# KELVIN-ASU/Lightweight-Multi-Modal-Scene-Understanding-via-Knowledge-Distillation

Measured on AMD Instinct MI355X. Metric: PandaSet 2-class KD training frames/sec, higher is better.
Workload: dtype f32; 1 GPU; KD step: concat-fusion teacher fwd (eval) -> weighted-fusion student fwd/bwd (train BN), CE + T^2*KL(T=4) + feature-MSE, fused AdamW; random-init weights; teacher_fusion=concat, student_fusion=weighted, image=3x256x256, points_per_frame=80000, bev_grid=64x64, num_classes=2, per_gpu_batch=256, global_batch=256, parallelism=dp1

## Files before the change

lightweight-multi-modal-scene-understanding-via-knowledge-distillation_amd/csrc/kd_lidar.hip:

```cpp
#include "kd_common.h"

namespace {

struct BevGeom { float x0, xd, y0, yd; int H, W; };

__device__ __forceinline__ bool bev_cell(const float4 pt, const BevGeom g, int& cell) {
  const float xn = __fdiv_rn(__fsub_rn(pt.x, g.x0), g.xd);
  const float yn = __fdiv_rn(__fsub_rn(pt.y, g.y0), g.yd);
  const bool valid = (xn >= 0.f) && (xn <= 1.f) && (yn >= 0.f) && (yn <= 1.f);
  if (!valid) { cell = -1; return false; }
  long long ix = (long long)__fmul_rn(xn, (float)(g.W - 1));
  long long iy = (long long)__fmul_rn(yn, (float)(g.H - 1));
  ix = ix < 0 ? 0 : (ix > g.W - 1 ? g.W - 1 : ix);
  iy = iy < 0 ? 0 : (iy > g.H - 1 ? g.H - 1 : iy);
  cell = (int)(iy * g.W + ix);
  return true;
}

struct L0Args {
  const float* pts; const float* w; const float* b; float* y; float* partial;
  int64_t P; int C; int groups, slots; const int* p_dev;
};
__global__ __launch_bounds__(256) void lidar_l0_fwd_kernel(L0Args a) {
  __shared__ float red[2 * 256 * 4];
// ... 290 lines not shown
  if (lane == 0) wave_cnt[wave] = __popcll(m);
  __syncthreads();
  if (threadIdx.x == 0) {
    int tot = 0;
    for (int w = 0; w < (int)(blockDim.x >> 6); ++w) { wave_off[w] = tot; tot += wave_cnt[w]; }
    block_base = tot ? atomicAdd(counter, tot) : 0;
  }
  __syncthreads();
  if (valid) {
    const int idx = block_base + wave_off[wave] + before;
    kd_st4(out_pts + (int64_t)idx * 4, pt);
    out_cell[idx] = (int)(p / N) * (g.H * g.W) + c;
  }
}
int kd_lidar_compact(const float* pts, float* out_pts, int* out_cell, int* counter, int B, int64_t N, int H, int W,
                     float x0, float x1, float y0, float y1, void* stream) {
  KD_REQUIRE(pts && out_pts && out_cell && counter && B > 0 && N > 0, KD_ERR_ARG, "kd_lidar_compact: bad args");
  hipStream_t st = (hipStream_t)stream;
  hipError_t e = kd_fill_async(counter, 0, sizeof(int), st);
  KD_REQUIRE(e == hipSuccess, (int)e, "kd_lidar_compact: memset failed: %s", hipGetErrorString(e));
  const int64_t P = (int64_t)B * N;
  hipLaunchKernelGGL(lidar_compact_kernel, dim3((unsigned)((P + 1023) / 1024)), dim3(1024), 0, st, pts, out_pts, out_cell,
                     counter, P, N, BevGeom{x0, x1 - x0, y0, y1 - y0, H, W});
  return kd_check_launch("kd_lidar_compact");
}

__global__ __launch_bounds__(256) void scatter_max_idx_kernel(const float* __restrict__ y, const float* __restrict__ sc,
                                                              const float* __restrict__ sh, int act,
                                                              const int* __restrict__ cell_idx, float* grid, int64_t P, int C,
                                                              int groups, int slots, const int* p_dev) {
  const int tid = threadIdx.x;
  const int gidx = tid % groups, slot = tid / groups;
  if (slot >= slots) return;
  const int G = groups;
  float s[4], h[4];
#pragma unroll
  for (int j = 0; j < 4; ++j) { s[j] = sc[gidx + G * j]; h[j] = sh[gidx + G * j]; }
  if (p_dev) { const int64_t pv = *p_dev; P = pv < P ? pv : P; }
  for (int64_t p = (int64_t)blockIdx.x * slots + slot; p < P; p += (int64_t)gridDim.x * slots) {
    const float* yp = y + p * C + gidx;
    unsigned* dst = reinterpret_cast<unsigned*>(grid + (int64_t)cell_idx[p] * C + gidx);
    float v[4];
    unsigned cur[4];
#pragma unroll
    for (int j = 0; j < 4; ++j) { v[j] = kd_act(kd_affine(yp[G * j], s[j], h[j]), act); cur[j] = dst[G * j]; }
#pragma unroll
    for (int j = 0; j < 4; ++j) {
      const unsigned u = __float_as_uint(v[j]);
      if (v[j] > 0.f && u > cur[j]) atomicMax(dst + G * j, u);
    }
  }
}
int kd_lidar_scatter_max_idx_fwd(const float* y, const float* sc, const float* sh, int act, const int* cell_idx,
                                 float* grid, int64_t P, int C, int64_t ncells, const int* p_dev, void* stream) {
  KD_REQUIRE(y && sc && sh && cell_idx && grid && P >= 0 && C % 4 == 0 && C <= 1024 && ncells > 0, KD_ERR_ARG, "kd_lidar_scatter_max_idx_fwd: bad args");
  KD_REQUIRE(act == KD_ACT_RELU || act == KD_ACT_RELU6, KD_ERR_ARG, "kd_lidar_scatter_max_idx_fwd: needs a non-negative activation");
  hipStream_t st = (hipStream_t)stream;
  hipError_t e = kd_fill_async(grid, 0, (size_t)ncells * C * sizeof(float), st);
  KD_REQUIRE(e == hipSuccess, (int)e, "kd_lidar_scatter_max_idx_fwd: memset failed: %s", hipGetErrorString(e));
  if (P == 0) return KD_OK;
  const KdCgLayout l = kd_cg_layout(P, C, 4096);
  hipLaunchKernelGGL(scatter_max_idx_kernel, dim3(l.grid), dim3(256), 0, st, y, sc, sh, act, cell_idx, grid, P, C, l.groups,
                     l.slots, p_dev);
  return kd_check_launch("kd_lidar_scatter_max_idx_fwd");
}

}

namespace {

constexpr int SCAN_CHUNK = 2048;

__global__ void seg_count_kernel(const float* __restrict__ pts, int* __restrict__ row_of_point, int* __restrict__ rank,
                                 int* counts, int64_t P, int64_t N, BevGeom g) {
  const int64_t p = (int64_t)blockIdx.x * blockDim.x + threadIdx.x;
  if (p >= P) return;
  int c;
  if (bev_cell(kd_ld4(pts + p * 4), g, c)) {
    const int row = (int)(p / N) * (g.H * g.W) + c;
    row_of_point[p] = row;
    rank[p] = atomicAdd(counts + row, 1);
  } else {
    row_of_point[p] = -1;
  }
}

__global__ __launch_bounds__(256) void scan_block_sums_kernel(const int* __restrict__ v, int* __restrict__ bsum, int64_t n) {
  __shared__ int red[256];
  const int64_t base = (int64_t)blockIdx.x * SCAN_CHUNK;
  int s = 0;
  for (int i = threadIdx.x; i < SCAN_CHUNK; i += 256)
    if (base + i < n) s += v[base + i];
  red[threadIdx.x] = s;
  __syncthreads();
  for (int off = 128; off > 0; off >>= 1) {
    if ((int)threadIdx.x < off) red[threadIdx.x] += red[threadIdx.x + off];
    __syncthreads();
  }
  if (threadIdx.x == 0) bsum[blockIdx.x] = red[0];
}

__global__ __launch_bounds__(1024) void scan_bsums_kernel(int* bsum, int nb) {
  __shared__ int sh[1024];
  int carry = 0;
  for (int base = 0; base < nb; base += 1024) {
    const int i = base + (int)threadIdx.x;
    const int v = i < nb ? bsum[i] : 0;
    sh[threadIdx.x] = v;
    __syncthreads();
    for (int off = 1; off < 1024; off <<= 1) {
      const int t = (int)threadIdx.x >= off ? sh[threadIdx.x - off] : 0;
      __syncthreads();
      sh[threadIdx.x] += t;
      __syncthreads();
    }
    if (i < nb) bsum[i] = carry + sh[threadIdx.x] - v;
    carry += sh[1023];
    __syncthreads();
  }
}

__global__ __launch_bounds__(256) void scan_apply_kernel(int* v, const int* __restrict__ bsum, int64_t n) {
  __shared__ int sh[256];
  const int64_t base = (int64_t)blockIdx.x * SCAN_CHUNK + (int64_t)threadIdx.x * 8;
  int x[8];
  int tot = 0;
#pragma unroll
  for (int j = 0; j < 8; ++j) { x[j] = base + j < n ? v[base + j] : 0; tot += x[j]; }
  sh[threadIdx.x] = tot;
  __syncthreads();
  for (int off = 1; off < 256; off <<= 1) {
    const int t = (int)threadIdx.x >= off ? sh[threadIdx.x - off] : 0;
    __syncthreads();
    sh[threadIdx.x] += t;
    __syncthreads();
  }
  int run = bsum[blockIdx.x] + sh[threadIdx.x] - tot;
#pragma unroll
  for (int j = 0; j < 8; ++j) {
    if (base + j < n) v[base + j] = run;
    run += x[j];
  }
}

__global__ void seg_fill_kernel(const int* __restrict__ row_of_point, const int* __restrict__ rank,
                                const int* __restrict__ start, int* __restrict__ perm, int64_t P) {
  const int64_t p = (int64_t)blockIdx.x * blockDim.x + threadIdx.x;
  if (p >= P) return;
  const int row = row_of_point[p];
  if (row >= 0) perm[start[row] + rank[p]] = (int)p;
}

constexpr int SORT_BLK = 1024;
constexpr int SORT_MAX_BINS = 36865;

__global__ __launch_bounds__(SORT_BLK) void stable_count_kernel(const float* __restrict__ pts, int* __restrict__ key_out,
                                                                int* __restrict__ lrank_out, int* __restrict__ T, int64_t N,
                                                                int nblk, BevGeom g) {
  extern __shared__ int hist[];
  const int HW = g.H * g.W, nb = HW + 1;
  const int tid = threadIdx.x, lane = tid & 63, wave = tid >> 6;
  const int b = blockIdx.x / nblk, blk = blockIdx.x % nblk;
  for (int i = tid; i < nb; i += SORT_BLK) hist[i] = 0;
  const int64_t n = (int64_t)blk * SORT_BLK + tid;
  const bool act = n < N;
  const int64_t p = (int64_t)b * N + (act ? n : 0);
  int key = -1;
  if (act) {
    int c;
    key = bev_cell(kd_ld4(pts + p * 4), g, c) ? c : HW;
  }
  int r = 0, cnt = 0;
#pragma unroll 16
  for (int j = 0; j < 64; ++j) {
    const int kj = __shfl(key, j);
    cnt += kj == key ? 1 : 0;
    r += (kj == key && j < lane) ? 1 : 0;
  }
  __syncthreads();
  int lr = 0;
  for (int w = 0; w < SORT_BLK / 64; ++w) {
    if (wave == w && act) lr = hist[key] + r;
    __syncthreads();
    if (wave == w && act && r == cnt - 1) hist[key] += cnt;
    __syncthreads();
  }
  if (act) { key_out[p] = key; lrank_out[p] = lr; }
  int* Tb = T + ((int64_t)b * nblk + blk) * nb;
  for (int i = tid; i < nb; i += SORT_BLK) Tb[i] = hist[i];
}

__global__ void stable_prefix_kernel(int* T, int* __restrict__ counts, int* __restrict__ inv, int B, int nblk, int HW) {
  const int nb = HW + 1;
  const int64_t idx = (int64_t)blockIdx.x * blockDim.x + threadIdx.x;
  if (idx == 0) counts[(int64_t)B * HW] = 0;
  if (idx >= (int64_t)B * nb) return;
  const int b = (int)(idx / nb), key = (int)(idx % nb);
  int run = 0;
  for (int blk = 0; blk < nblk; ++blk) {
    int* t = T + ((int64_t)b * nblk + blk) * nb + key;
    const int v = *t;
    *t = run;
    run += v;
  }
  if (key < HW) counts[(int64_t)b * HW + key] = run; else inv[b] = run;
}

__global__ void stable_inv_base_kernel(const int* __restrict__ seg_start, int* inv, int B, int64_t ncells) {
  if (threadIdx.x != 0 || blockIdx.x != 0) return;
  int run = seg_start[ncells];
  for (int b = 0; b < B; ++b) { const int v = inv[b]; inv[b] = run; run += v; }
}

__global__ void stable_fill_kernel(const float* __restrict__ pts, const int* __restrict__ key, const int* __restrict__ lrank,
                                   const int* __restrict__ T, const int* __restrict__ seg_start, const int* __restrict__ inv_base,
                                   float* __restrict__ pts_sorted, int* __restrict__ row_sorted, int* __restrict__ perm,
                                   int64_t P, int64_t N, int nblk, int HW) {
  const int64_t p = (int64_t)blockIdx.x * blockDim.x + threadIdx.x;
  if (p >= P) return;
  const int b = (int)(p / N), blk = (int)((p % N) / SORT_BLK), k = key[p];
  const int base = k < HW ? seg_start[(int64_t)b * HW + k] : inv_base[b];
  const int64_t pos = (int64_t)base + T[((int64_t)b * nblk + blk) * (HW + 1) + k] + lrank[p];
  kd_st4(pts_sorted + pos * 4, kd_ld4(pts + p * 4));
  row_sorted[pos] = k < HW ? b * HW + k : -1;
  if (perm) perm[pos] = (int)p;
}

constexpr int WIDE_MAX_DIM = 4096;

__device__ __forceinline__ void wave_same_key(int key, int lane, int& below, int& all) {
  below = 0; all = 0;
#pragma unroll 16
  for (int j = 0; j < 64; ++j) {
    const int kj = __shfl(key, j);
    all += kj == key ? 1 : 0;
    below += (kj == key && j < lane) ? 1 : 0;
  }
}

__device__ __forceinline__ int block_stable_rank(int key, bool act, int below, int all, int* hist) {
  const int wave = threadIdx.x >> 6;
  int lr = 0;
  for (int w = 0; w < SORT_BLK / 64; ++w) {
    if (wave == w && act) lr = hist[key] + below;
    __syncthreads();
    if (wave == w && act && below == all - 1) hist[key] += all;
    __syncthreads();
  }
  return lr;
}

template <int PASS>
__global__ __launch_bounds__(SORT_BLK) void wide_count_kernel(const float* __restrict__ pts, int* __restrict__ cell_io,
                                                              int* __restrict__ lrank_out, int* __restrict__ T,
                                                              int* counts, int64_t N, int nblk, BevGeom g) {
  extern __shared__ int hist[];
  const int nd = PASS == 0 ? g.W : g.H + 1;
  const int tid = threadIdx.x, lane = tid & 63;
  const int b = blockIdx.x / nblk, blk = blockIdx.x % nblk;
  for (int i = tid; i < nd; i += SORT_BLK) hist[i] = 0;
  const int64_t n = (int64_t)blk * SORT_BLK + tid;
  const bool act = n < N;
  const int64_t p = (int64_t)b * N + (act ? n : 0);
  int cell = -1;
  if (act) {
    if (PASS == 0) bev_cell(kd_ld4(pts + p * 4), g, cell); else cell = cell_io[p];
  }
  const int key = !act ? -1 : PASS == 0 ? (cell >= 0 ? cell % g.W : 0) : (cell >= 0 ? cell / g.W : g.H);
  int below, all;
  wave_same_key(key, lane, below, all);
  if (PASS == 0) {
    int cbelow, call;
    wave_same_key(cell, lane, cbelow, call);
    if (cell >= 0 && cbelow == 0) atomicAdd(counts + (int64_t)b * g.H * g.W + cell, call);
  }
  __syncthreads();
  const int lr = block_stable_rank(key, act, below, all, hist);
  if (act) {
    if (PASS == 0) cell_io[p] = cell;
    lrank_out[p] = lr;
  }
  int* Tb = T + ((int64_t)b * nblk + blk) * nd;
  for (int i = tid; i < nd; i += SORT_BLK) Tb[i] = hist[i];
}

__global__ void wide_prefix_kernel(int* T, int* __restrict__ tot, int* __restrict__ last_tot, int B, int nblk, int nd) {
  const int64_t idx = (int64_t)blockIdx.x * blockDim.x + threadIdx.x;
  if (idx >= (int64_t)B * nd) return;
  const int b = (int)(idx / nd), d = (int)(idx % nd);
  int run = 0;
  for (int blk = 0; blk < nblk; ++blk) {
    int* t = T + ((int64_t)b * nblk + blk) * nd + d;
    const int v = *t;
    *t = run;
    run += v;
  }
  tot[idx] = run;
  if (last_tot && d == nd - 1) last_tot[b] = run;
}

__global__ __launch_bounds__(64) void wide_frame_scan_kernel(int* tot, int nd) {
  int* t = tot + (int64_t)blockIdx.x * nd;
  const int lane = threadIdx.x;
  int carry = 0;
  for (int base = 0; base < nd; base += 64) {
    const int i = base + lane;
    const int v = i < nd ? t[i] : 0;
    int incl = v;
#pragma unroll
    for (int off = 1; off < 64; off <<= 1) {
      const int u = __shfl_up(incl, off);
      if (lane >= off) incl += u;
    }
    if (i < nd) t[i] = carry + incl - v;
    carry += __shfl(incl, 63);
  }
}

__global__ void wide_mid_kernel(const int* __restrict__ cell, const int* __restrict__ lrank, const int* __restrict__ T,
                                const int* __restrict__ off, int* __restrict__ mid_id, int* __restrict__ mid_cell, int64_t P,
                                int64_t N, int nblk, int W) {
  const int64_t p = (int64_t)blockIdx.x * blockDim.x + threadIdx.x;
  if (p >= P) return;
  const int b = (int)(p / N), blk = (int)((p % N) / SORT_BLK), c = cell[p];
  const int d = c >= 0 ? c % W : 0;
  const int64_t pos = (int64_t)b * N + off[(int64_t)b * W + d] + T[((int64_t)b * nblk + blk) * W + d] + lrank[p];
  mid_id[pos] = (int)p;
  mid_cell[pos] = c;
}

__global__ void wide_fill_kernel(const float* __restrict__ pts, const int* __restrict__ mid_id, const int* __restrict__ mid_cell,
                                 const int* __restrict__ lrank, const int* __restrict__ T, const int* __restrict__ off,
                                 const int* __restrict__ seg_start, const int* __restrict__ inv_base,
                                 float* __restrict__ pts_sorted, int* __restrict__ row_sorted, int* __restrict__ perm,
                                 int64_t P, int64_t N, int nblk, int H, int W) {
  const int64_t q = (int64_t)blockIdx.x * blockDim.x + threadIdx.x;
  if (q >= P) return;
  const int b = (int)(q / N), blk = (int)((q % N) / SORT_BLK), c = mid_cell[q], p = mid_id[q];
  const int nd = H + 1, d = c >= 0 ? c / W : H;
  const int64_t HW = (int64_t)H * W;
  const int in_digit = T[((int64_t)b * nblk + blk) * nd + d] + lrank[q];
  const int64_t pos = c >= 0 ? (int64_t)seg_start[b * HW] + off[(int64_t)b * nd + d] + in_digit : (int64_t)inv_base[b] + in_digit;
  kd_st4(pts_sorted + pos * 4, kd_ld4(pts + (int64_t)p * 4));
  row_sorted[pos] = c >= 0 ? (int)(b * HW + c) : -1;
  if (perm) perm[pos] = p;
}

struct SegArgs {
  const float* y; const float* sc; const float* sh; int act;
  const int* start; const int* perm;
  float* grid; const float* dout; const float* mean; const float* invstd;
  float* G; float* partial; int64_t ncells; int C;
  int long_len; const int* rowid; float* cnt; int prow0;
  float* rawmax; uint8_t* holders;
};
constexpr int SEG_LONG = 256;
constexpr int SEG_HOLD_SWEEP = 255;

template <int VEC> struct SegVec;
template <> struct SegVec<1> { typedef float type; };
template <> struct SegVec<2> { typedef float2 type; };
template <> struct SegVec<4> { typedef float4 type; };

template <int VEC> __device__ __forceinline__ void seg_ld(float (&r)[VEC], const float* p) {
  const typename SegVec<VEC>::type v = *reinterpret_cast<const typename SegVec<VEC>::type*>(p);
  __builtin_memcpy(r, &v, sizeof(v));
}
template <int VEC> __device__ __forceinline__ void seg_st(float* p, const float (&r)[VEC]) {
  typename SegVec<VEC>::type v;
  __builtin_memcpy(&v, r, sizeof(v));
  *reinterpret_cast<typename SegVec<VEC>::type*>(p) = v;
}

template <int VEC, bool PERM>
__global__ __launch_bounds__(256) void seg_max_fwd_kernel(SegArgs a) {
  const int lane = threadIdx.x & 63;
// ... 305 lines not shown
  const int nvalid = __builtin_amdgcn_readfirstlane(a.start[a.ncells]);
  const int64_t nw = (int64_t)gridDim.x * 4;
  for (int64_t w = (int64_t)blockIdx.x * 4 + wave; w * 64 < nvalid; w += nw) {
    const int i0 = (int)(w * 64), i1 = i0 + 64 < nvalid ? i0 + 64 : nvalid;
    const int cf = __builtin_amdgcn_readfirstlane(a.rowid[i0]), cl = __builtin_amdgcn_readfirstlane(a.rowid[i1 - 1]);
    const bool lf = a.start[cf + 1] - a.start[cf] > a.long_len, ll = a.start[cl + 1] - a.start[cl] > a.long_len;
    if (!lf && !ll) continue;
    int i = i0;
    while (i < i1) {
      const int cell = __builtin_amdgcn_readfirstlane(a.rowid[i]);
      const int cs = __builtin_amdgcn_readfirstlane(a.start[cell]), ce = __builtin_amdgcn_readfirstlane(a.start[cell + 1]);
      const int rend = ce < i1 ? ce : i1;
      if (ce - cs <= a.long_len) { i = rend; continue; }
      float acc[VEC], mx[VEC], share[VEC];
#pragma unroll
      for (int j = 0; j < VEC; ++j) { acc[j] = 0.f; mx[j] = 0.f; share[j] = 0.f; }
      if (MODE >= 1) seg_ld<VEC>(mx, a.grid + (int64_t)cell * a.C + c0);
      if (MODE == 2) {
        float d[VEC], n[VEC];
        seg_ld<VEC>(d, a.dout + (int64_t)cell * a.C + c0);
        seg_ld<VEC>(n, a.cnt + (int64_t)cell * a.C + c0);
#pragma unroll
        for (int j = 0; j < VEC; ++j) share[j] = n[j] > 0.f ? d[j] / n[j] : 0.f;
        if (i == cs) seg_st<VEC>(a.G + (int64_t)cell * a.C + c0, share);
      }
      int k = i;
      for (; k + 4 <= rend; k += 4) {
        float r[4][VEC];
#pragma unroll
        for (int u = 0; u < 4; ++u) seg_ld<VEC>(r[u], a.y + (int64_t)(k + u) * a.C + c0);
#pragma unroll
        for (int u = 0; u < 4; ++u)
#pragma unroll
          for (int j = 0; j < VEC; ++j) {
            const float v = kd_act(kd_affine(r[u][j], sc[j], sh[j]), a.act);
            if (MODE == 0) acc[j] = v > acc[j] ? v : acc[j];
            if (MODE == 1) acc[j] += (v > 0.f && v == mx[j]) ? 1.f : 0.f;
            if (MODE == 2) {
              const float g = (v > 0.f && v == mx[j]) ? share[j] : 0.f;
              s1[j] += g;
              s2[j] = fmaf(g, (r[u][j] - mu[j]) * inv[j], s2[j]);
            }
          }
      }
      for (; k < rend; ++k) {
        float r[VEC];
        seg_ld<VEC>(r, a.y + (int64_t)k * a.C + c0);
#pragma unroll
        for (int j = 0; j < VEC; ++j) {
          const float v = kd_act(kd_affine(r[j], sc[j], sh[j]), a.act);
          if (MODE == 0) acc[j] = v > acc[j] ? v : acc[j];
          if (MODE == 1) acc[j] += (v > 0.f && v == mx[j]) ? 1.f : 0.f;
          if (MODE == 2) {
            const float g = (v > 0.f && v == mx[j]) ? share[j] : 0.f;
            s1[j] += g;
            s2[j] = fmaf(g, (r[j] - mu[j]) * inv[j], s2[j]);
          }
        }
      }
      if (MODE == 0) {
        unsigned* dst = reinterpret_cast<unsigned*>(a.grid + (int64_t)cell * a.C + c0);
#pragma unroll
        for (int j = 0; j < VEC; ++j)
          if (acc[j] > 0.f) atomicMax(dst + j, __float_as_uint(acc[j]));
      }
      if (MODE == 1) {
#pragma unroll
        for (int j = 0; j < VEC; ++j)
          if (acc[j] > 0.f) atomicAdd(a.cnt + (int64_t)cell * a.C + c0 + j, acc[j]);
      }
      i = rend;
    }
  }
  if (MODE == 2) {
#pragma unroll
    for (int j = 0; j < VEC; ++j) { red[wave][0][c0 + j] = s1[j]; red[wave][1][c0 + j] = s2[j]; }
    __syncthreads();
    for (int i = threadIdx.x; i < 2 * a.C; i += 256) {
      const int st = i / a.C, c = i % a.C;
      a.partial[((int64_t)(a.prow0 + blockIdx.x) * 2 + st) * a.C + c] = red[0][st][c] + red[1][st][c] + red[2][st][c] + red[3][st][c];
    }
  }
}

inline int seg_long_grid(int64_t P) { const int64_t b = (P + 255) / 256; return (int)(b < 1024 ? b : 1024); }

__global__ __launch_bounds__(256) void seg_zero_invalid_kernel(const int* __restrict__ row_of_point, float* __restrict__ G,
                                                               int64_t P, int c4) {
  const int per = 256 / c4;
  const int q = threadIdx.x % c4, sub = threadIdx.x / c4;
  const int64_t base = (int64_t)blockIdx.x * per * 16;
#pragma unroll 4
  for (int k = 0; k < 16; ++k) {
    const int64_t p = base + (int64_t)k * per + sub;
    if (p < P && row_of_point[p] < 0) kd_st4(G + (p * c4 + q) * 4, kd_zero4());
  }
}

__global__ void seg_gather_kernel(const float* __restrict__ pts, const int* __restrict__ perm, const int* __restrict__ row_of_point,
                                  const int* __restrict__ nvalid, float* __restrict__ out_pts, int* __restrict__ out_row, int64_t P) {
  const int64_t i = (int64_t)blockIdx.x * blockDim.x + threadIdx.x;
  if (i >= P || i >= *nvalid) return;
  const int p = perm[i];
  kd_st4(out_pts + i * 4, kd_ld4(pts + (int64_t)p * 4));
  out_row[i] = row_of_point[p];
}

inline int seg_grid(int64_t ncells) { const int64_t b = (ncells + 3) / 4; return (int)(b < 4096 ? b : 4096); }

}

extern "C" {

size_t kd_lidar_cell_sort_ws_bytes(int B, int64_t N, int H, int W) {
  const int64_t n = (int64_t)B * H * W + 1;
  return ((size_t)B * N + (size_t)((n + SCAN_CHUNK - 1) / SCAN_CHUNK)) * sizeof(int);
}

int kd_lidar_cell_sort(const float* pts, int B, int64_t N, int H, int W, float x0, float x1, float y0, float y1,
                       int* row_of_point, int* seg_start, int* perm, void* ws, size_t ws_bytes, void* stream) {
  KD_REQUIRE(pts && row_of_point && seg_start && perm && ws && B > 0 && N > 0 && H > 0 && W > 0, KD_ERR_ARG, "kd_lidar_cell_sort: bad args");
  const int64_t P = (int64_t)B * N, n = (int64_t)B * H * W + 1;
  KD_REQUIRE(P < (int64_t)INT32_MAX && n < (int64_t)INT32_MAX, KD_ERR_SHAPE, "kd_lidar_cell_sort: more than 2^31 points or cells");
  KD_REQUIRE(ws_bytes >= kd_lidar_cell_sort_ws_bytes(B, N, H, W), KD_ERR_WORKSPACE, "kd_lidar_cell_sort: workspace too small");
  hipStream_t st = (hipStream_t)stream;
  int* rank = (int*)ws;
  int* bsum = rank + P;
  const int nb = (int)((n + SCAN_CHUNK - 1) / SCAN_CHUNK);
  hipError_t e = kd_fill_async(seg_start, 0, (size_t)n * sizeof(int), st);
  KD_REQUIRE(e == hipSuccess, (int)e, "kd_lidar_cell_sort: memset failed: %s", hipGetErrorString(e));
  const BevGeom g{x0, x1 - x0, y0, y1 - y0, H, W};
  hipLaunchKernelGGL(seg_count_kernel, dim3((unsigned)((P + 255) / 256)), dim3(256), 0, st, pts, row_of_point, rank, seg_start, P, N, g);
  hipLaunchKernelGGL(scan_block_sums_kernel, dim3(nb), dim3(256), 0, st, seg_start, bsum, n);
  hipLaunchKernelGGL(scan_bsums_kernel, dim3(1), dim3(1024), 0, st, bsum, nb);
  hipLaunchKernelGGL(scan_apply_kernel, dim3(nb), dim3(256), 0, st, seg_start, bsum, n);
  hipLaunchKernelGGL(seg_fill_kernel, dim3((unsigned)((P + 255) / 256)), dim3(256), 0, st, row_of_point, rank, seg_start, perm, P);
  return kd_check_launch("kd_lidar_cell_sort");
}

size_t kd_lidar_sort_points_ws_bytes(int B, int64_t N, int H, int W) {
  const int64_t P = (int64_t)B * N, nblk = (N + SORT_BLK - 1) / SORT_BLK, nb = (int64_t)H * W + 1, n = (int64_t)B * H * W + 1;
  return (size_t)(2 * P + (int64_t)B * nblk * nb + B + (n + SCAN_CHUNK - 1) / SCAN_CHUNK) * sizeof(int);
}

int kd_lidar_sort_points(const float* pts, int B, int64_t N, int H, int W, float x0, float x1, float y0, float y1,
                         float* pts_sorted, int* row_sorted, int* seg_start, int* perm, void* ws, size_t ws_bytes,
                         void* stream) {
  KD_REQUIRE(pts && pts_sorted && row_sorted && seg_start && ws && B > 0 && N > 0 && H > 0 && W > 0, KD_ERR_ARG, "kd_lidar_sort_points: bad args");
  const int64_t P = (int64_t)B * N, ncells = (int64_t)B * H * W, n = ncells + 1;
  const int HW = H * W, nb = HW + 1;
  KD_REQUIRE(nb <= SORT_MAX_BINS, KD_ERR_SHAPE, "kd_lidar_sort_points: H*W + 1 = %d bins exceed %d", nb, SORT_MAX_BINS);
  KD_REQUIRE(P < (int64_t)INT32_MAX && n < (int64_t)INT32_MAX, KD_ERR_SHAPE, "kd_lidar_sort_points: more than 2^31 points or cells");
  KD_REQUIRE(ws_bytes >= kd_lidar_sort_points_ws_bytes(B, N, H, W), KD_ERR_WORKSPACE, "kd_lidar_sort_points: workspace too small");
  const int nblk = (int)((N + SORT_BLK - 1) / SORT_BLK);
  KD_REQUIRE((int64_t)B * nblk < (int64_t)INT32_MAX, KD_ERR_SHAPE, "kd_lidar_sort_points: too many blocks");
  hipStream_t st = (hipStream_t)stream;
  int* key = (int*)ws;
  int* lrank = key + P;
  int* T = lrank + P;
  int* inv = T + (int64_t)B * nblk * nb;
  int* bsum = inv + B;
  const int nsb = (int)((n + SCAN_CHUNK - 1) / SCAN_CHUNK);
  const BevGeom g{x0, x1 - x0, y0, y1 - y0, H, W};
  if ((size_t)nb * sizeof(int) > 48 * 1024) {
    hipError_t e = hipFuncSetAttribute(reinterpret_cast<const void*>(stable_count_kernel), hipFuncAttributeMaxDynamicSharedMemorySize,
                                       SORT_MAX_BINS * (int)sizeof(int));
    KD_REQUIRE(e == hipSuccess, (int)e, "kd_lidar_sort_points: cannot raise the LDS limit: %s", hipGetErrorString(e));
  }
  hipLaunchKernelGGL(stable_count_kernel, dim3((unsigned)(B * nblk)), dim3(SORT_BLK), (size_t)nb * sizeof(int), st, pts, key, lrank, T,
                     N, nblk, g);
  const int64_t nbk = (int64_t)B * nb;
  hipLaunchKernelGGL(stable_prefix_kernel, dim3((unsigned)((nbk + 255) / 256)), dim3(256), 0, st, T, seg_start, inv, B, nblk, HW);
  hipLaunchKernelGGL(scan_block_sums_kernel, dim3(nsb), dim3(256), 0, st, seg_start, bsum, n);
  hipLaunchKernelGGL(scan_bsums_kernel, dim3(1), dim3(1024), 0, st, bsum, nsb);
  hipLaunchKernelGGL(scan_apply_kernel, dim3(nsb), dim3(256), 0, st, seg_start, bsum, n);
  hipLaunchKernelGGL(stable_inv_base_kernel, dim3(1), dim3(64), 0, st, seg_start, inv, B, ncells);
  hipLaunchKernelGGL(stable_fill_kernel, dim3((unsigned)((P + 255) / 256)), dim3(256), 0, st, pts, key, lrank, T, seg_start, inv,
                     pts_sorted, row_sorted, perm, P, N, nblk, HW);
  return kd_check_launch("kd_lidar_sort_points");
}

size_t kd_lidar_sort_points_wide_ws_bytes(int B, int64_t N, int H, int W) {
  const int64_t P = (int64_t)B * N, nblk = (N + SORT_BLK - 1) / SORT_BLK, n = (int64_t)B * H * W + 1, nd = (int64_t)W + H + 1;
  return (size_t)(4 * P + (int64_t)B * nblk * nd + (int64_t)B * nd + B + (n + SCAN_CHUNK - 1) / SCAN_CHUNK) * sizeof(int);
}

int kd_lidar_sort_points_wide(const float* pts, int B, int64_t N, int H, int W, float x0, float x1, float y0, float y1,
                              float* pts_sorted, int* row_sorted, int* seg_start, int* perm, void* ws, size_t ws_bytes,
                              void* stream) {
  KD_REQUIRE(pts && pts_sorted && row_sorted && seg_start && ws && B > 0 && N > 0 && H > 0 && W > 0, KD_ERR_ARG, "kd_lidar_sort_points_wide: bad args");
  KD_REQUIRE(H <= WIDE_MAX_DIM && W <= WIDE_MAX_DIM, KD_ERR_SHAPE, "kd_lidar_sort_points_wide: grid %d x %d exceeds %d cells per side", H, W,
             WIDE_MAX_DIM);
  const int64_t P = (int64_t)B * N, ncells = (int64_t)B * H * W, n = ncells + 1;
  KD_REQUIRE(P < (int64_t)INT32_MAX && n < (int64_t)INT32_MAX, KD_ERR_SHAPE, "kd_lidar_sort_points_wide: more than 2^31 points or cells");
  KD_REQUIRE(ws_bytes >= kd_lidar_sort_points_wide_ws_bytes(B, N, H, W), KD_ERR_WORKSPACE, "kd_lidar_sort_points_wide: workspace too small");
  const int nblk = (int)((N + SORT_BLK - 1) / SORT_BLK);
  KD_REQUIRE((int64_t)B * nblk < (int64_t)INT32_MAX, KD_ERR_SHAPE, "kd_lidar_sort_points_wide: too many blocks");
  hipStream_t st = (hipStream_t)stream;
  const int nd0 = W, nd1 = H + 1;
  int* cell = (int*)ws;
  int* lrank = cell + P;
  int* mid_id = lrank + P;
  int* mid_cell = mid_id + P;
  int* T0 = mid_cell + P;
  int* T1 = T0 + (int64_t)B * nblk * nd0;
  int* off0 = T1 + (int64_t)B * nblk * nd1;
  int* off1 = off0 + (int64_t)B * nd0;
  int* inv = off1 + (int64_t)B * nd1;
  int* bsum = inv + B;
  const int nsb = (int)((n + SCAN_CHUNK - 1) / SCAN_CHUNK);
  const BevGeom g{x0, x1 - x0, y0, y1 - y0, H, W};
  hipError_t e = kd_fill_async(seg_start, 0, (size_t)n * sizeof(int), st);
  KD_REQUIRE(e == hipSuccess, (int)e, "kd_lidar_sort_points_wide: memset failed: %s", hipGetErrorString(e));
  const dim3 blocks((unsigned)(B * nblk)), per_point((unsigned)((P + 255) / 256));
  hipLaunchKernelGGL(wide_count_kernel<0>, blocks, dim3(SORT_BLK), (size_t)nd0 * sizeof(int), st, pts, cell, lrank, T0, seg_start, N, nblk, g);
  hipLaunchKernelGGL(wide_prefix_kernel, dim3((unsigned)(((int64_t)B * nd0 + 255) / 256)), dim3(256), 0, st, T0, off0, (int*)nullptr, B, nblk, nd0);
  hipLaunchKernelGGL(wide_frame_scan_kernel, dim3(B), dim3(64), 0, st, off0, nd0);
  hipLaunchKernelGGL(wide_mid_kernel, per_point, dim3(256), 0, st, cell, lrank, T0, off0, mid_id, mid_cell, P, N, nblk, W);
  hipLaunchKernelGGL(wide_count_kernel<1>, blocks, dim3(SORT_BLK), (size_t)nd1 * sizeof(int), st, (const float*)nullptr, mid_cell, lrank, T1,
                     (int*)nullptr, N, nblk, g);
  hipLaunchKernelGGL(wide_prefix_kernel, dim3((unsigned)(((int64_t)B * nd1 + 255) / 256)), dim3(256), 0, st, T1, off1, inv, B, nblk, nd1);
  hipLaunchKernelGGL(wide_frame_scan_kernel, dim3(B), dim3(64), 0, st, off1, nd1);
  hipLaunchKernelGGL(scan_block_sums_kernel, dim3(nsb), dim3(256), 0, st, seg_start, bsum, n);
  hipLaunchKernelGGL(scan_bsums_kernel, dim3(1), dim3(1024), 0, st, bsum, nsb);
  hipLaunchKernelGGL(scan_apply_kernel, dim3(nsb), dim3(256), 0, st, seg_start, bsum, n);
  hipLaunchKernelGGL(stable_inv_base_kernel, dim3(1), dim3(64), 0, st, seg_start, inv, B, ncells);
  hipLaunchKernelGGL(wide_fill_kernel, per_point, dim3(256), 0, st, pts, mid_id, mid_cell, lrank, T1, off1, seg_start, inv, pts_sorted,
                     row_sorted, perm, P, N, nblk, H, W);
  return kd_check_launch("kd_lidar_sort_points_wide");
}

int kd_lidar_gather_sorted(const float* pts, const int* perm, const int* row_of_point, const int* nvalid_dev, float* out_pts,
                           int* out_row, int64_t P, void* stream) {
  KD_REQUIRE(pts && perm && row_of_point && nvalid_dev && out_pts && out_row && P > 0, KD_ERR_ARG, "kd_lidar_gather_sorted: bad args");
  hipLaunchKernelGGL(seg_gather_kernel, dim3((unsigned)((P + 255) / 256)), dim3(256), 0, (hipStream_t)stream, pts, perm, row_of_point,
                     nvalid_dev, out_pts, out_row, P);
  return kd_check_launch("kd_lidar_gather_sorted");
}

int kd_lidar_seg_max_fwd(const float* y, const float* sc, const float* sh, int act, const int* seg_start, const int* perm,
                         const int* row_sorted, float* grid, int64_t P, int64_t ncells, int C, void* stream) {
  KD_REQUIRE(y && sc && sh && seg_start && grid && ncells > 0, KD_ERR_ARG, "kd_lidar_seg_max_fwd: bad args");
  KD_REQUIRE(C == 64 || C == 128 || C == 256, KD_ERR_SHAPE, "kd_lidar_seg_max_fwd: C must be 64, 128 or 256 (got %d)", C);
  KD_REQUIRE(act == KD_ACT_RELU || act == KD_ACT_RELU6, KD_ERR_ARG, "kd_lidar_seg_max_fwd: needs a non-negative activation");
  const bool chunked = row_sorted != nullptr && perm == nullptr && P > 0;
  SegArgs a{y, sc, sh, act, seg_start, perm, grid, nullptr, nullptr, nullptr, nullptr, nullptr, ncells, C,
            chunked ? SEG_LONG : 0, row_sorted, nullptr, 0};
  const dim3 gr(seg_grid(ncells)), bl(256);
  hipStream_t st = (hipStream_t)stream;
#define KD_SEG_LAUNCH(kern)                                                                          \
  do {                                                                                              \
    if (C == 64) { if (perm) hipLaunchKernelGGL((kern<1, true>), gr, bl, 0, st, a); else hipLaunchKernelGGL((kern<1, false>), gr, bl, 0, st, a); } \
    else if (C == 128) { if (perm) hipLaunchKernelGGL((kern<2, true>), gr, bl, 0, st, a); else hipLaunchKernelGGL((kern<2, false>), gr, bl, 0, st, a); } \
    else { if (perm) hipLaunchKernelGGL((kern<4, true>), gr, bl, 0, st, a); else hipLaunchKernelGGL((kern<4, false>), gr, bl, 0, st, a); } \
  } while (0)
  KD_SEG_LAUNCH(seg_max_fwd_kernel);
  if (chunked) {
    const dim3 gl(seg_long_grid(P));
    if (C == 64) hipLaunchKernelGGL((seg_long_kernel<1, 0>), gl, bl, 0, st, a);
    else if (C == 128) hipLaunchKernelGGL((seg_long_kernel<2, 0>), gl, bl, 0, st, a);
    else hipLaunchKernelGGL((seg_long_kernel<4, 0>), gl, bl, 0, st, a);
  }
  return kd_check_launch("kd_lidar_seg_max_fwd");
}

int64_t kd_lidar_seg_stat_rows(int64_t ncells) { return seg_grid(ncells); }

int kd_lidar_seg_max_bwd(const float* y, const float* sc, const float* sh, int act, const float* grid, const float* dout,
                         const float* mean, const float* invstd, const int* seg_start, const int* perm,
                         const int* row_of_point, float* G, float* partial, int64_t P, int64_t ncells, int C, void* stream) {
  KD_REQUIRE(y && sc && sh && grid && dout && mean && invstd && seg_start && row_of_point && G && partial && P > 0 && ncells > 0,
             KD_ERR_ARG, "kd_lidar_seg_max_bwd: bad args");
  KD_REQUIRE(act != KD_ACT_RELU6, KD_ERR_ARG, "kd_lidar_seg_max_bwd: ReLU6 is not supported in the scatter-max backward (a saturated maximum has derivative 0; the holder split here is ReLU's)");
  KD_REQUIRE(C == 64 || C == 128 || C == 256, KD_ERR_SHAPE, "kd_lidar_seg_max_bwd: C must be 64, 128 or 256 (got %d)", C);
  SegArgs a{y, sc, sh, act, seg_start, perm, const_cast<float*>(grid), dout, mean, invstd, G, partial, ncells, C, 0, nullptr, nullptr, 0};
  const dim3 gr(seg_grid(ncells)), bl(256);
  hipStream_t st = (hipStream_t)stream;
  const int c4 = C / 4;
  const int64_t per_block = (int64_t)(256 / c4) * 16;
  hipLaunchKernelGGL(seg_zero_invalid_kernel, dim3((unsigned)((P + per_block - 1) / per_block)), dim3(256), 0, st, row_of_point, G, P, c4);
  KD_SEG_LAUNCH(seg_max_bwd_kernel);
#undef KD_SEG_LAUNCH
  return kd_check_launch("kd_lidar_seg_max_bwd");
}

int64_t kd_lidar_seg_share_stat_rows(int64_t ncells, int64_t P) { return seg_grid(ncells) + seg_long_grid(P); }

int kd_lidar_seg_share_bwd(const float* y, const float* sc, const float* sh, int act, const float* grid, const float* dout,
                           const float* mean, const float* invstd, const int* seg_start, const int* row_sorted, float* share,
                           float* cnt_ws, float* partial, int64_t P, int64_t ncells, int C, void* stream) {
  KD_REQUIRE(y && sc && sh && grid && dout && mean && invstd && seg_start && row_sorted && share && cnt_ws && partial && ncells > 0 && P > 0,
             KD_ERR_ARG, "kd_lidar_seg_share_bwd: bad args");
  KD_REQUIRE(act != KD_ACT_RELU6, KD_ERR_ARG, "kd_lidar_seg_share_bwd: ReLU6 is not supported in the scatter-max backward (a saturated maximum has derivative 0; the holder split here is ReLU's)");
  KD_REQUIRE(C == 64 || C == 128 || C == 256, KD_ERR_SHAPE, "kd_lidar_seg_share_bwd: C must be 64, 128 or 256 (got %d)", C);
  SegArgs a{y, sc, sh, act, seg_start, nullptr, const_cast<float*>(grid), dout, mean, invstd, share, partial, ncells, C,
            SEG_LONG, row_sorted, cnt_ws, seg_grid(ncells)};
  const dim3 gr(seg_grid(ncells)), gl(seg_long_grid(P)), bl(256);
  hipStream_t st = (hipStream_t)stream;
  if (C == 64) {
    hipLaunchKernelGGL((seg_max_bwd_kernel<1, false, true>), gr, bl, 0, st, a);
    hipLaunchKernelGGL((seg_long_kernel<1, 1>), gl, bl, 0, st, a);
    hipLaunchKernelGGL((seg_long_kernel<1, 2>), gl, bl, 0, st, a);
  } else if (C == 128) {
    hipLaunchKernelGGL((seg_max_bwd_kernel<2, false, true>), gr, bl, 0, st, a);
    hipLaunchKernelGGL((seg_long_kernel<2, 1>), gl, bl, 0, st, a);
    hipLaunchKernelGGL((seg_long_kernel<2, 2>), gl, bl, 0, st, a);
  } else {
    hipLaunchKernelGGL((seg_max_bwd_kernel<4, false, true>), gr, bl, 0, st, a);
    hipLaunchKernelGGL((seg_long_kernel<4, 1>), gl, bl, 0, st, a);
    hipLaunchKernelGGL((seg_long_kernel<4, 2>), gl, bl, 0, st, a);
  }
  return kd_check_launch("kd_lidar_seg_share_bwd");
}

int kd_lidar_seg_hold_fwd(const float* y, const float* sc, const float* sh, int act, const int* seg_start, const int* row_sorted,
                          float* grid, float* rawmax, uint8_t* holders, int64_t P, int64_t ncells, int C, void* stream) {
  KD_REQUIRE(y && sc && sh && seg_start && row_sorted && grid && rawmax && holders && ncells > 0 && P > 0, KD_ERR_ARG,
             "kd_lidar_seg_hold_fwd: bad args");
  KD_REQUIRE(C == 64 || C == 128 || C == 256, KD_ERR_SHAPE, "kd_lidar_seg_hold_fwd: C must be 64, 128 or 256 (got %d)", C);
  KD_REQUIRE(act == KD_ACT_RELU || act == KD_ACT_RELU6, KD_ERR_ARG, "kd_lidar_seg_hold_fwd: needs a non-negative activation");
  KD_REQUIRE((uintptr_t)holders % 4 == 0, KD_ERR_ARG, "kd_lidar_seg_hold_fwd: holders must be 4-byte aligned");
  SegArgs a{y, sc, sh, act, seg_start, nullptr, grid, nullptr, nullptr, nullptr, nullptr, nullptr, ncells, C,
            SEG_LONG, row_sorted, nullptr, 0, rawmax, holders};
  const dim3 gr(seg_grid(ncells)), gl(seg_long_grid(P)), bl(256);
  hipStream_t st = (hipStream_t)stream;
  if (C == 64) {
    hipLaunchKernelGGL((seg_hold_fwd_kernel<1>), gr, bl, 0, st, a);
    hipLaunchKernelGGL((seg_long_kernel<1, 0>), gl, bl, 0, st, a);
  } else if (C == 128) {
    hipLaunchKernelGGL((seg_hold_fwd_kernel<2>), gr, bl, 0, st, a);
    hipLaunchKernelGGL((seg_long_kernel<2, 0>), gl, bl, 0, st, a);
// ... 38 lines not shown
```

Before: 3658 frames/s.

## Tile stable count sort over 8 points per thread and recompute keys in fill

Measured after the change: 3675 frames/s, median of 6. No clear change (+0.5%).

```diff
diff --git a/lightweight-multi-modal-scene-understanding-via-knowledge-distillation_amd/csrc/kd_lidar.hip b/lightweight-multi-modal-scene-understanding-via-knowledge-distillation_amd/csrc/kd_lidar.hip
--- a/lightweight-multi-modal-scene-understanding-via-knowledge-distillation_amd/csrc/kd_lidar.hip
+++ b/lightweight-multi-modal-scene-understanding-via-knowledge-distillation_amd/csrc/kd_lidar.hip
@@ -466,40 +466,55 @@
 }
 
 constexpr int SORT_BLK = 1024;
+constexpr int SORT_PPT = 8;
+constexpr int SORT_TILE = SORT_BLK * SORT_PPT;
 constexpr int SORT_MAX_BINS = 36865;
 
-__global__ __launch_bounds__(SORT_BLK) void stable_count_kernel(const float* __restrict__ pts, int* __restrict__ key_out,
-                                                                int* __restrict__ lrank_out, int* __restrict__ T, int64_t N,
-                                                                int nblk, BevGeom g) {
+__global__ __launch_bounds__(SORT_BLK) __attribute__((amdgpu_waves_per_eu(8)))
+void stable_count_kernel(const float* __restrict__ pts, int* __restrict__ lrank_out, int* __restrict__ T, int64_t N, int nblk,
+                         BevGeom g) {
   extern __shared__ int hist[];
   const int HW = g.H * g.W, nb = HW + 1;
   const int tid = threadIdx.x, lane = tid & 63, wave = tid >> 6;
   const int b = blockIdx.x / nblk, blk = blockIdx.x % nblk;
   for (int i = tid; i < nb; i += SORT_BLK) hist[i] = 0;
-  const int64_t n = (int64_t)blk * SORT_BLK + tid;
-  const bool act = n < N;
-  const int64_t p = (int64_t)b * N + (act ? n : 0);
-  int key = -1;
-  if (act) {
-    int c;
-    key = bev_cell(kd_ld4(pts + p * 4), g, c) ? c : HW;
-  }
-  int r = 0, cnt = 0;
+  const int64_t n0 = (int64_t)blk * SORT_TILE + tid;
+  int keys[SORT_PPT];
+#pragma unroll
+  for (int t = 0; t < SORT_PPT; ++t) {
+    const int64_t n = n0 + t * SORT_BLK;
+    keys[t] = -1;
+    if (n < N) {
+      int c;
+      keys[t] = bev_cell(kd_ld4(pts + ((int64_t)b * N + n) * 4), g, c) ? c : HW;
+    }
+  }
+  __syncthreads();
+  int lrs[SORT_PPT] = {};
+#pragma unroll
+  for (int t = 0; t < SORT_PPT; ++t) {
+    if ((int64_t)blk * SORT_TILE + t * SORT_BLK >= N) break;
+    const int key = keys[t];
+    const bool act = key >= 0;
+    int r = 0, cnt = 0;
 #pragma unroll 16
-  for (int j = 0; j < 64; ++j) {
-    const int kj = __shfl(key, j);
-    cnt += kj == key ? 1 : 0;
-    r += (kj == key && j < lane) ? 1 : 0;
-  }
-  __syncthreads();
-  int lr = 0;
-  for (int w = 0; w < SORT_BLK / 64; ++w) {
-    if (wave == w && act) lr = hist[key] + r;
-    __syncthreads();
-    if (wave == w && act && r == cnt - 1) hist[key] += cnt;
-    __syncthreads();
-  }
-  if (act) { key_out[p] = key; lrank_out[p] = lr; }
+    for (int j = 0; j < 64; ++j) {
+      const int kj = __shfl(key, j);
+      cnt += kj == key ? 1 : 0;
+      r += (kj == key && j < lane) ? 1 : 0;
+    }
+    for (int w = 0; w < SORT_BLK / 64; ++w) {
+      if (wave == w && act) {
+        const int lr = hist[key] + r;
+        if (r == cnt - 1) hist[key] = lr + 1;
+        lrs[t] = lr;
+      }
+      __syncthreads();
+    }
+  }
+#pragma unroll
+  for (int t = 0; t < SORT_PPT; ++t)
+    if (keys[t] >= 0) lrank_out[(int64_t)b * N + n0 + t * SORT_BLK] = lrs[t];
   int* Tb = T + ((int64_t)b * nblk + blk) * nb;
   for (int i = tid; i < nb; i += SORT_BLK) Tb[i] = hist[i];
 }
@@ -520,22 +535,41 @@
   if (key < HW) counts[(int64_t)b * HW + key] = run; else inv[b] = run;
 }
 
-__global__ void stable_inv_base_kernel(const int* __restrict__ seg_start, int* inv, int B, int64_t ncells) {
-  if (threadIdx.x != 0 || blockIdx.x != 0) return;
-  int run = seg_start[ncells];
-  for (int b = 0; b < B; ++b) { const int v = inv[b]; inv[b] = run; run += v; }
-}
-
-__global__ void stable_fill_kernel(const float* __restrict__ pts, const int* __restrict__ key, const int* __restrict__ lrank,
-                                   const int* __restrict__ T, const int* __restrict__ seg_start, const int* __restrict__ inv_base,
-                                   float* __restrict__ pts_sorted, int* __restrict__ row_sorted, int* __restrict__ perm,
-                                   int64_t P, int64_t N, int nblk, int HW) {
-  const int64_t p = (int64_t)blockIdx.x * blockDim.x + threadIdx.x;
-  if (p >= P) return;
-  const int b = (int)(p / N), blk = (int)((p % N) / SORT_BLK), k = key[p];
+__global__ __launch_bounds__(64) void stable_inv_base_kernel(const int* __restrict__ seg_start, int* inv, int B, int64_t ncells) {
+  const int lane = threadIdx.x;
+  int carry = seg_start[ncells];
+  for (int base = 0; base < B; base += 64) {
+    const int i = base + lane;
+    const int v = i < B ? inv[i] : 0;
+    int incl = v;
+#pragma unroll
+    for (int off = 1; off < 64; off <<= 1) {
+      const int u = __shfl_up(incl, off);
+      if (lane >= off) incl += u;
+    }
+    if (i < B) inv[i] = carry + incl - v;
+    carry += __shfl(incl, 63);
+  }
+}
+
+__global__ __launch_bounds__(256) void stable_fill_kernel(const float* __restrict__ pts, const int* __restrict__ lrank,
+                                                          const int* __restrict__ T, const int* __restrict__ seg_start,
+                                                          const int* __restrict__ inv_base, float* __restrict__ pts_sorted,
+                                                          int* __restrict__ row_sorted, int* __restrict__ perm, int B,
+                                                          int64_t N, int nblk, BevGeom g) {
+  const int fb = (int)((N + 255) / 256);
+  const int x = blockIdx.x % 8, j = blockIdx.x / 8;
+  const int b = j / fb * 8 + x;
+  const int64_t n = (int64_t)(j % fb) * 256 + threadIdx.x;
+  if (b >= B || n >= N) return;
+  const int64_t p = (int64_t)b * N + n;
+  const int HW = g.H * g.W, blk = (int)(n / SORT_TILE);
+  const float4 pt = kd_ld4(pts + p * 4);
+  int c;
+  const int k = bev_cell(pt, g, c) ? c : HW;
   const int base = k < HW ? seg_start[(int64_t)b * HW + k] : inv_base[b];
   const int64_t pos = (int64_t)base + T[((int64_t)b * nblk + blk) * (HW + 1) + k] + lrank[p];
-  kd_st4(pts_sorted + pos * 4, kd_ld4(pts + p * 4));
+  kd_st4(pts_sorted + pos * 4, pt);
   row_sorted[pos] = k < HW ? b * HW + k : -1;
   if (perm) perm[pos] = (int)p;
 }
@@ -1147,11 +1181,11 @@
   KD_REQUIRE(nb <= SORT_MAX_BINS, KD_ERR_SHAPE, "kd_lidar_sort_points: H*W + 1 = %d bins exceed %d", nb, SORT_MAX_BINS);
   KD_REQUIRE(P < (int64_t)INT32_MAX && n < (int64_t)INT32_MAX, KD_ERR_SHAPE, "kd_lidar_sort_points: more than 2^31 points or cells");
   KD_REQUIRE(ws_bytes >= kd_lidar_sort_points_ws_bytes(B, N, H, W), KD_ERR_WORKSPACE, "kd_lidar_sort_points: workspace too small");
-  const int nblk = (int)((N + SORT_BLK - 1) / SORT_BLK);
-  KD_REQUIRE((int64_t)B * nblk < (int64_t)INT32_MAX, KD_ERR_SHAPE, "kd_lidar_sort_points: too many blocks");
+  const int nblk = (int)((N + SORT_TILE - 1) / SORT_TILE);
+  const int64_t fill_blocks = ((int64_t)B + 7) / 8 * 8 * ((N + 255) / 256);
+  KD_REQUIRE((int64_t)B * nblk < (int64_t)INT32_MAX && fill_blocks < (int64_t)INT32_MAX, KD_ERR_SHAPE, "kd_lidar_sort_points: too many blocks");
   hipStream_t st = (hipStream_t)stream;
-  int* key = (int*)ws;
-  int* lrank = key + P;
+  int* lrank = (int*)ws;
   int* T = lrank + P;
   int* inv = T + (int64_t)B * nblk * nb;
   int* bsum = inv + B;
@@ -1162,16 +1196,16 @@
                                        SORT_MAX_BINS * (int)sizeof(int));
     KD_REQUIRE(e == hipSuccess, (int)e, "kd_lidar_sort_points: cannot raise the LDS limit: %s", hipGetErrorString(e));
   }
-  hipLaunchKernelGGL(stable_count_kernel, dim3((unsigned)(B * nblk)), dim3(SORT_BLK), (size_t)nb * sizeof(int), st, pts, key, lrank, T,
-                     N, nblk, g);
+  hipLaunchKernelGGL(stable_count_kernel, dim3((unsigned)(B * nblk)), dim3(SORT_BLK), (size_t)nb * sizeof(int), st, pts, lrank, T, N, nblk,
+                     g);
   const int64_t nbk = (int64_t)B * nb;
   hipLaunchKernelGGL(stable_prefix_kernel, dim3((unsigned)((nbk + 255) / 256)), dim3(256), 0, st, T, seg_start, inv, B, nblk, HW);
   hipLaunchKernelGGL(scan_block_sums_kernel, dim3(nsb), dim3(256), 0, st, seg_start, bsum, n);
   hipLaunchKernelGGL(scan_bsums_kernel, dim3(1), dim3(1024), 0, st, bsum, nsb);
   hipLaunchKernelGGL(scan_apply_kernel, dim3(nsb), dim3(256), 0, st, seg_start, bsum, n);
   hipLaunchKernelGGL(stable_inv_base_kernel, dim3(1), dim3(64), 0, st, seg_start, inv, B, ncells);
-  hipLaunchKernelGGL(stable_fill_kernel, dim3((unsigned)((P + 255) / 256)), dim3(256), 0, st, pts, key, lrank, T, seg_start, inv,
-                     pts_sorted, row_sorted, perm, P, N, nblk, HW);
+  hipLaunchKernelGGL(stable_fill_kernel, dim3((unsigned)fill_blocks), dim3(256), 0, st, pts, lrank, T, seg_start, inv, pts_sorted,
+                     row_sorted, perm, B, N, nblk, g);
   return kd_check_launch("kd_lidar_sort_points");
 }
 
```
